# ishine/pix2pixHDAudioSR

Hardware: AMD Instinct MI355X
Metric: MDCT spectrogram frames/sec (G+D fwd+bwd) at 512x256 (higher is better)
Workload: dtype bf16; 1 GPU; configs[1]: ngf=48 n_local_enhancers=0 (GlobalGenerator nd4 nb9) + MultiscaleDiscriminator num_D=2, 512x256 MDCT4 (n_fft 1024, hop 512), LSGAN + feature matching, Adam, bf16 MFMA; per_gpu_batch=32, global_batch=32, parallelism=dp1, launch=hip-graph replay

## Files before the change

pix2pixhdaudiosr_amd/csrc/convplan.h:

```cpp
#pragma once
#include "common.h"
#include <algorithm>

namespace p2phd {

struct GDesc {
  int N, Hin, Win, Cp_in;
  int Hg, Wg;
  int sh, sw, pad_mode;
  int rx_base;
  int Hout, Wout, Cp_out;
  int oh_mul, oh_off, ow_mul, ow_off;
  int Kout, KK, act;
  int nth, ntw, dh0, dh_step, dw0, dw_step;
  int wr0, wr_step, ws0, ws_step;
  int flat_m;
  int cw_inject;
  int cls_cp;
  int n_extent;
  int cls_skip;
  unsigned in_bytes, w_bytes;
  int stats_slots;
  const float* out_scale;
  const void* bs_y;
  const float* bs_stats;
  float* bs_out;
  float bs_inv_hw, bs_eps, bs_slope;
  const void* as_x;
  int grid_m, sk_first, sk_tail, sk_parts, sk_steps;
  float* sk_part;
  unsigned* sk_ticket;
};

struct WMap {
  int rows, inner;
  long s_row, s_inner;
  int row_mod; long s_rowq;
  int c_mod; long s_innerq;
  int S;
  long s_tap;
};
inline WMap plain_map(int rows, int inner, long s_row, long s_inner, int S, long s_tap = 1) {
  return WMap{rows, inner, s_row, s_inner, rows > 0 ? rows : 1, 0, inner > 0 ? inner : 1, 0, S, s_tap};
}

constexpr int P2PHD_FP8_INTERNAL = 2;
int launch_pack_fp8(const GDesc& d, const WMap& m, const float* w, void* wp8, int rows_pad, float* scale2, unsigned* amax_bits,
                    hipStream_t st);

enum LaunchFamily { LC_GCONV = 0, LC_HALO, LC_CLS_SKIP, LC_MARCH, LC_MARCH_W, LC_WGRAD, LC_SPLITK, LC_TILE256, LC_TILE128X192,
                    LC_DFIRST, LC_DLAST, LC_C7, LC_THIN_WGRAD, LC_TIMED_PACK, LC_TIMED_FRAMES, LC_STITCH, LC_PCM, LC_METRICS_ROWS,
                    LC_XOVER, LC_SPECIMG, LC_LOUDNESS, LC_TRUEPEAK, LC_LIMITER, LC_BANDWIDTH, LC_STEREO, LC_RATECONV, LC_FAMILIES };
extern unsigned long long g_launch_count[LC_FAMILIES];

int pcm_check_rows(const char* what, int64_t frames, int channels, int64_t ld, int format, bool encodable);

extern int g_opt_gconv_bm;
extern int g_opt_wgrad_tm;
extern int g_opt_tile128x192;
extern int g_opt_wgrad_xcd;
extern int g_opt_c7_generic;
extern int g_opt_splitk_tail;
extern int g_opt_truepeak_grid;
extern int g_opt_limiter_grid;
extern int g_opt_cus;
int device_cus();
extern int g_opt_reflect_generic;
extern int g_opt_c7_abl;

struct BSum { const void* y; const float* stats; float* out; float inv_hw, eps, slope; };
bool c7_in_shape_ok(const p2phd_conv_desc* c);
size_t c7_in_packed_elems(const p2phd_conv_desc* c);
int c7_in_pack(const p2phd_conv_desc* c, const float* w, void* wf, hipStream_t st);
int c7_in_slots(const p2phd_conv_desc* c);
int c7_in_fwd(const p2phd_conv_desc* c, const void* x, const void* wf, const float* bias, void* y, float* table, hipStream_t st);
bool c7_out_shape_ok(const p2phd_conv_desc* c);
size_t c7_out_packed_elems(const p2phd_conv_desc* c);
int c7_out_pack(const p2phd_conv_desc* c, const float* w, void* wf, hipStream_t st);
int c7_out_fwd(const p2phd_conv_desc* c, const void* x, const void* wf, const float* bias, int act, void* y, hipStream_t st);
bool c7_dgrad_shape_ok(const p2phd_conv_desc* c);
size_t c7_out_dgrad_packed_elems(const p2phd_conv_desc* c);
int c7_out_dgrad_pack(const p2phd_conv_desc* c, const float* w, void* wf, hipStream_t st);
int c7_out_dgrad(const p2phd_conv_desc* c, const void* dy, const void* wf, const float* w_master, void* dx, hipStream_t st);
extern int g_opt_dfirst;
bool dfirst_shape_ok(const p2phd_conv_desc* c);
size_t dfirst_packed_elems(const p2phd_conv_desc* c);
int dfirst_pack(const p2phd_conv_desc* c, const float* w, void* wf, hipStream_t st);
int dfirst_fwd(const p2phd_conv_desc* c, const void* x, const void* wf, const float* bias, int act, void* y, hipStream_t st);
extern int g_opt_dlast;
bool dlast_shape_ok(const p2phd_conv_desc* c);
size_t dlast_packed_elems(const p2phd_conv_desc* c, int which);
int dlast_pack(const p2phd_conv_desc* c, int which, const float* w, void* wfrag, hipStream_t st);
size_t dlast_fwd_workspace_floats(const p2phd_conv_desc* c);
int dlast_fwd(const p2phd_conv_desc* c, const void* x, const void* wf, const float* bias, void* y, float* part, hipStream_t st);
void dlast_dgrad_plan(const p2phd_conv_desc* c, int* bpw, int* slots);
size_t dlast_bsum_table_floats(const p2phd_conv_desc* c);
int dlast_dgrad(const p2phd_conv_desc* c, const void* dy, const void* wg, const void* addend, void* dx, const BSum* bs, hipStream_t st);
extern int g_opt_march; extern int g_opt_cls_skip; extern int g_opt_gconv_halo; extern int g_opt_cw_inject;
int march_shape_kind(const p2phd_conv_desc* c, int which);
size_t march_packed_elems(const p2phd_conv_desc* c, int which);
int march_pack(const p2phd_conv_desc* c, int which, const float* w, void* wf, hipStream_t st);
void march_plan(const p2phd_conv_desc* c, int which, int* slots, int* ncls, int* slot_rows, long* npix_cls, int* bs_tiles);
int march_run(const p2phd_conv_desc* c, int which, const void* in, const void* wf, const float* bias, void* out, float* table,
              const BSum* bs, hipStream_t st, const float* in_stats = nullptr, float in_slope = 1.f, float in_eps = 0.f);
size_t march_w_workspace_floats(const p2phd_conv_desc* c);
int march_w_run(const p2phd_conv_desc* c, const void* x, const void* dy, float* dw, int accumulate, const float* x_stats, float x_slope,
                float x_eps, float* slabs, hipStream_t st);
int thin_wgrad_shape_kind(const p2phd_conv_desc* c);
size_t thin_wgrad_workspace_floats(const p2phd_conv_desc* c);
int thin_wgrad(const p2phd_conv_desc* c, const void* x, const void* dy, float* dw, int accumulate, float* slabs, hipStream_t st);

inline int cpitch(int c) { return (c + 7) & ~7; }
inline int round_up(int v, int m) { return (v + m - 1) / m * m; }

int launch_gconv(const GDesc& d, int dtype, const void* in, const void* wp, const float* bias, const void* addend,
                 void* out, float* stats, hipStream_t st, int* slot_rows = nullptr);
struct GconvTile { int bm, bn, mr, nr, nstage, halo, flat_m; };
GconvTile gconv_choose_tile(const GDesc& d, int dtype, bool stats_wanted);
constexpr int kGconvRows256 = 256, kGconvCols192 = 192;
long gconv_mtiles256(const GDesc& d, bool flat_m);
bool gconv_256x192_fills_chip(const GDesc& d, bool flat_m);
inline int gconv_slot_rows(int bm, int mr, bool fused_sums) { return fused_sums ? bm : mr * 32; }
inline size_t stat_table_floats(const GDesc& d) {
  return (size_t)d.N * ((d.Hg * d.Wg + 31) / 32) * (d.cls_cp > 0 ? 4 : 1) * d.Cp_out * 2;
}
inline size_t bsum_table_floats(const GDesc& d) {
  const size_t tiles = ((size_t)d.Hg * d.Wg + 127) / 128;
  return (size_t)d.N * tiles * (size_t)(d.n_extent ? d.n_extent : d.Cp_out) * 2;
}
int launch_bsum_merge(const float* table, float* bstats, int N, long npix, int tile_rows, int n_extent, int cls_cp, int Cp, int C,
                      hipStream_t st);
int launch_stats_merge(const float* table, float* stats, int N, int slots, int ncls, int Cp, int C, long npix, int slot_rows,
                       hipStream_t st);
size_t wgrad_workspace_floats(const GDesc& d, int dtype, int M_rows, int M_rows_pad);
int launch_wgrad(const GDesc& d, const WMap& m, int dtype, const void* rows, int Cp_r, int M_rows, int M_rows_pad,
                 const void* gat, float* dwp, float* dw, int accumulate, hipStream_t st);
void launch_unpack_grad(const GDesc& d, const WMap& m, const float* dwp, float* dw, int splits, long slab_elems, int accumulate,
                        hipStream_t st);
int launch_pack_merged(const GDesc& d, int dtype, const float* w, void* wp, int rows_pad, int K, int C, int R, int S, int pad,
                       long s_k, long s_c, hipStream_t st);
int launch_pack(const GDesc& d, const WMap& m, int dtype, const float* w, void* wp, int rows_pad, hipStream_t st);
int launch_reflect_expand(int dtype, const void* dy, void* e_out, int N, int H, int W, int Cp, hipStream_t st);
// ... 14 lines not shown
```

pix2pixhdaudiosr_amd/csrc/core.hip:

```cpp
#include "common.h"
#include "convplan.h"
#include <cstring>

namespace p2phd {
static thread_local char g_err[512] = "";
void set_error(const char* fmt, ...) {
  va_list ap;
  va_start(ap, fmt);
  vsnprintf(g_err, sizeof(g_err), fmt, ap);
  va_end(ap);
}
}

namespace p2phd { int g_opt_gconv_bm = 0; int g_opt_wgrad_tm = 0; int g_opt_wgrad_xcd = 1; int g_opt_march = 1; int g_opt_cls_skip = 1; int g_opt_gconv_halo = 1; int g_opt_cw_inject = 0; int g_opt_tile128x192 = 1; int g_opt_mdct_generic = 0; int g_opt_mdct_iters = 0; int g_opt_c7_generic = 0; int g_opt_dfirst = 1; int g_opt_dlast = 1; int g_opt_c7_abl = 0; int g_opt_reflect_generic = 0; int g_opt_splitk_tail = 1; int g_opt_truepeak_grid = 0; int g_opt_limiter_grid = 0; int g_opt_cus = 0;
unsigned long long g_launch_count[LC_FAMILIES] = {};
int device_cus() {
  static int cached[64] = {};
  int dev = 0;
  if (hipGetDevice(&dev) != hipSuccess || dev < 0 || dev >= 64) return 256;
  if (cached[dev] == 0) {
    hipDeviceProp_t prop;
    cached[dev] = hipGetDeviceProperties(&prop, dev) == hipSuccess ? prop.multiProcessorCount : 256;
  }
  return cached[dev];
}
}

namespace {
constexpr int kFoldRegions = 9;
constexpr size_t kFoldFloats[kFoldRegions] = {size_t(4) << 20, size_t(1) << 20, size_t(1) << 20, 4096, size_t(16) << 20, size_t(5) << 16, size_t(1) << 16, size_t(1) << 16, 0};
constexpr int kFoldTickets[kFoldRegions] = {2048, 1024, 8, 8, 256, 8, 8, 8, 1024};
constexpr int kFoldTicketsAll = 2048 + 1024 + 16 + 256 + 8 + 8 + 8 + 1024;
__device__ float g_fold_part[(size_t(22) << 20) + 4096 + (size_t(7) << 16)];
__device__ unsigned g_fold_ticket[kFoldTicketsAll];
}
namespace p2phd {
namespace {
struct FoldDev { float* part = nullptr; unsigned* ticket = nullptr; hipStream_t last[kFoldRegions] = {}; bool used[kFoldRegions] = {}; hipEvent_t ev[kFoldRegions] = {}; bool ev_set[kFoldRegions] = {}; };
FoldDev g_fold_dev[64];
thread_local hipStream_t g_fold_pending_stream = nullptr;
FoldDev* fold_dev() {
  int dev = 0;
  if (hipGetDevice(&dev) != hipSuccess || dev < 0 || dev >= 64) return nullptr;
  FoldDev& f = g_fold_dev[dev];
  if (f.part == nullptr) {
    void* p = nullptr; void* t = nullptr;
    if (hipGetSymbolAddress(&p, HIP_SYMBOL(g_fold_part)) != hipSuccess || hipGetSymbolAddress(&t, HIP_SYMBOL(g_fold_ticket)) != hipSuccess)
      return nullptr;
    f.part = static_cast<float*>(p); f.ticket = static_cast<unsigned*>(t);
  }
  return &f;
}
bool capturing(hipStream_t s) {
  hipStreamCaptureStatus cs = hipStreamCaptureStatusNone;
  return hipStreamIsCapturing(s, &cs) == hipSuccess && cs == hipStreamCaptureStatusActive;
}
}

thread_local int g_fold_pending = -1;

FoldScratch fold_capacity(int region) {
  if (region < 0 || region >= kFoldRegions) return FoldScratch{nullptr, nullptr, 0, 0};
  return FoldScratch{nullptr, nullptr, kFoldFloats[region], kFoldTickets[region]};
}

FoldScratch fold_scratch(int region, hipStream_t stream) {
  FoldDev* f = fold_dev();
  if (f == nullptr || region < 0 || region >= kFoldRegions) { set_error("reduction scratch unavailable"); return FoldScratch{nullptr, nullptr, 0, 0}; }
  const bool cap = capturing(stream);
  if (f->used[region] && f->last[region] != stream && f->ev_set[region] && !cap) {
    if (hipStreamWaitEvent(stream, f->ev[region], 0) != hipSuccess) {
      (void)hipGetLastError();
      set_error("reduction-scratch region %d: cannot order this stream behind the region's previous launch "
                "(include/p2phd.h, \"Streams\")", region);
      return FoldScratch{nullptr, nullptr, 0, 0};
    }
  }
  f->used[region] = true;
  f->last[region] = stream;
  g_fold_pending = cap ? -1 : region;
  g_fold_pending_stream = stream;
  size_t fo = 0; int to = 0;
  for (int r = 0; r < region; ++r) { fo += kFoldFloats[r]; to += kFoldTickets[r]; }
  const FoldScratch cap_of = fold_capacity(region);
  return FoldScratch{f->part + fo, f->ticket + to, cap_of.floats, cap_of.tickets};
}

void fold_launched() {
  const int region = g_fold_pending;
  g_fold_pending = -1;
  FoldDev* f = fold_dev();
  if (f == nullptr || region < 0 || region >= kFoldRegions) return;
  if (f->ev[region] == nullptr && hipEventCreateWithFlags(&f->ev[region], hipEventDisableTiming) != hipSuccess) { (void)hipGetLastError(); f->ev[region] = nullptr; return; }
  if (hipEventRecord(f->ev[region], g_fold_pending_stream) == hipSuccess) f->ev_set[region] = true;
  else (void)hipGetLastError();
}
}

extern "C" int p2phd_reduction_reset(void* stream) {
  void* t = nullptr;
  if (hipGetSymbolAddress(&t, HIP_SYMBOL(g_fold_ticket)) != hipSuccess) { p2phd::set_error("reduction_reset: no device symbol"); return P2PHD_ELAUNCH; }
  if (hipMemsetAsync(t, 0, sizeof(unsigned) * kFoldTicketsAll, (hipStream_t)stream) != hipSuccess) {
    p2phd::set_error("reduction_reset: memset failed");
    return P2PHD_ELAUNCH;
  }
  return P2PHD_OK;
}

extern "C" int p2phd_set_option(const char* name, int value) {
  if (name && !strcmp(name, "gconv_bm") && (value == 0 || value == 128 || value == 192 || value == 256 || value == 258 || value == 512)) { p2phd::g_opt_gconv_bm = value; return P2PHD_OK; }
  if (name && !strcmp(name, "wgrad_tm") && (value == 0 || value == 128)) { p2phd::g_opt_wgrad_tm = value; return P2PHD_OK; }
  if (name && !strcmp(name, "march") && (value == 0 || value == 1)) { p2phd::g_opt_march = value; return P2PHD_OK; }
  if (name && !strcmp(name, "cls_skip") && (value == 0 || value == 1)) { p2phd::g_opt_cls_skip = value; return P2PHD_OK; }
  if (name && !strcmp(name, "gconv_halo") && (value == 0 || value == 1)) { p2phd::g_opt_gconv_halo = value; return P2PHD_OK; }
  if (name && !strcmp(name, "tile128x192") && (value == 0 || value == 1)) { p2phd::g_opt_tile128x192 = value; return P2PHD_OK; }
  if (name && !strcmp(name, "dlast") && (value == 0 || value == 1)) { p2phd::g_opt_dlast = value; return P2PHD_OK; }
  if (name && !strcmp(name, "dfirst") && (value == 0 || value == 1)) { p2phd::g_opt_dfirst = value; return P2PHD_OK; }
#ifdef P2PHD_CHECK_WAITS
  if (name && !strcmp(name, "cw_inject") && (value == 0 || value == 1)) { p2phd::g_opt_cw_inject = value; return P2PHD_OK; }
#endif
  if (name && !strcmp(name, "wgrad_xcd") && (value == 0 || value == 1)) { p2phd::g_opt_wgrad_xcd = value; return P2PHD_OK; }
  if (name && !strcmp(name, "reflect_generic") && (value == 0 || value == 1)) { p2phd::g_opt_reflect_generic = value; return P2PHD_OK; }
  if (name && !strcmp(name, "mdct_iters") && value >= 0 && value <= 8) { p2phd::g_opt_mdct_iters = value; return P2PHD_OK; }
  if (name && !strcmp(name, "splitk_tail") && value >= 0 && value <= 2) { p2phd::g_opt_splitk_tail = value; return P2PHD_OK; }
  if (name && !strcmp(name, "cus") && value >= 0 && value <= 4096) { p2phd::g_opt_cus = value; return P2PHD_OK; }
  if (name && !strcmp(name, "truepeak_grid") && value >= 0 && value <= 65536) { p2phd::g_opt_truepeak_grid = value; return P2PHD_OK; }
  if (name && !strcmp(name, "limiter_grid") && value >= 0 && value <= 16384) { p2phd::g_opt_limiter_grid = value; return P2PHD_OK; }
  if (name && !strcmp(name, "c7_abl")) { p2phd::g_opt_c7_abl = value; return P2PHD_OK; }
  if (name && !strcmp(name, "c7_generic") && (value == 0 || value == 1)) { p2phd::g_opt_c7_generic = value; return P2PHD_OK; }
  if (name && !strcmp(name, "mdct_generic") && (value == 0 || value == 1)) { p2phd::g_opt_mdct_generic = value; return P2PHD_OK; }
  p2phd::set_error("set_option: unknown option or value (%s = %d)", name ? name : "(null)", value);
  return P2PHD_EINVAL;
}

extern "C" int64_t p2phd_launch_count(const char* family, int reset) {
  static const char* names[p2phd::LC_FAMILIES] = {"gconv", "halo", "cls_skip", "march", "march_w", "wgrad", "splitk", "tile256", "tile128x192",
                                                       "dfirst", "dlast", "c7", "thin_wgrad", "timed_pack", "timed_frames", "stitch", "pcm",
                                                       "metrics_rows", "xover", "specimg", "loudness", "truepeak", "limiter", "bandwidth", "stereo", "rateconv"};
  if (family == nullptr) {
    if (reset) for (auto& c : p2phd::g_launch_count) c = 0;
    return 0;
  }
  for (int i = 0; i < p2phd::LC_FAMILIES; ++i)
    if (!strcmp(family, names[i])) {
      const int64_t v = (int64_t)p2phd::g_launch_count[i];
      if (reset) p2phd::g_launch_count[i] = 0;
      return v;
    }
  p2phd::set_error("launch_count: unknown kernel family %s", family);
  return -1;
}

extern "C" const char* p2phd_last_error(void) { return p2phd::g_err; }
extern "C" int p2phd_abi_version(void) { return 1; }
extern "C" int p2phd_half_type(void) {
#ifdef P2PHD_F16
  return 2;
#else
  return 1;
#endif
}

extern "C" int p2phd_device_info(char* name, int cap) {
  int dev = 0;
  if (hipGetDevice(&dev) != hipSuccess) {
    p2phd::set_error("no HIP device");
    return P2PHD_ELAUNCH;
  }
  hipDeviceProp_t prop;
  if (hipGetDeviceProperties(&prop, dev) != hipSuccess) {
    p2phd::set_error("hipGetDeviceProperties failed");
    return P2PHD_ELAUNCH;
  }
  if (name && cap > 0) {
    strncpy(name, prop.gcnArchName, cap - 1);
    name[cap - 1] = 0;
  }
  return prop.multiProcessorCount;
}
```

pix2pixhdaudiosr_amd/csrc/gconv.hip:

```cpp
#include "common.h"
#include "convplan.h"
#include "convdev.h"
#include "waitcheck.h"
#include <cmath>
#include <utility>
#include <vector>
#include <type_traits>

namespace {

using p2phd::GDesc;
using p2phd::GconvTile;

struct fp8_t { unsigned char v; };
template <> struct Elem<fp8_t> { static constexpr int EPP = 16; };
template <typename T> struct OutOf { typedef T type; };
template <> struct OutOf<fp8_t> { typedef bf16_t type; };

#ifdef P2PHD_PROBE
constexpr int kProbeSlots = 65536;
__device__ unsigned long long g_probe[kProbeSlots * 8];
#endif

template <typename T, int BM, int BN, int MR, int NR, int NSTAGE, int HALO = 0>
__global__ __launch_bounds__((BM / (MR * 32)) * (BN / (NR * 32)) * 64) void gconv_kernel(const GDesc d, const T* __restrict__ in, const T* __restrict__ wp,
                                                    const float* __restrict__ bias,
                                                    const typename OutOf<T>::type* __restrict__ addend,
                                                    typename OutOf<T>::type* __restrict__ out, float* __restrict__ stats) {
  typedef typename OutOf<T>::type TO;
  constexpr int EPPO = Elem<TO>::EPP;
  constexpr int EPP = Elem<T>::EPP;
  constexpr int BK = 8 * EPP;
  constexpr int WGM = BM / (MR * 32), WGN = BN / (NR * 32);
  constexpr int NT = WGM * WGN * 64;
  static_assert(NT == BM * 2 || NT == BM, "tile config");
  constexpr int STAGE = (BM + BN) * kRowBytes;
  constexpr int RS = NT / 8;
  constexpr int NB = BN * 8 / NT;
  constexpr int NA = BM * 8 / NT;
  static_assert(NB >= 1 && (NA == 4 || NA == 8), "piece distribution");
  constexpr int NLOADS = NA + NB;

  const int Cp = d.Cp_in, KK = d.KK, Wg = d.Wg, T_taps = d.nth * d.ntw, npix = d.Hg * d.Wg;
  const int Cp_out = d.Cp_out, Kout = d.Kout, act = d.act, cls_cp = d.cls_cp, n_extent = d.n_extent, stats_slots = d.stats_slots;

  extern __shared__ float4 smem_raw[];
  char* smem = reinterpret_cast<char*>(smem_raw);
  int* tab = reinterpret_cast<int*>(smem);
  int2* rinfo = reinterpret_cast<int2*>(smem + (HALO ? 0 : ((T_taps * BM * 4 + 15) & ~15)));
  char* stages = reinterpret_cast<char*>(rinfo + BM);
#ifdef P2PHD_PROBE
  const unsigned long long pr_t0 = __builtin_readcyclecounter();
#endif

  const int tid = threadIdx.x, lane = tid & 63;
  const int wave = __builtin_amdgcn_readfirstlane(tid >> 6);
  const int wm = wave / WGN, wn = wave % WGN;
  const bool flat = d.flat_m != 0;
  const int mtiles = (npix + BM - 1) / BM;
  int tile_id = (int)blockIdx.x, sk_part = -1, sk_tile = 0;
  if (tile_id >= d.sk_first) {
    const int r = tile_id - d.sk_first;
    sk_part = r / d.sk_tail;
    sk_tile = r - sk_part * d.sk_tail;
    tile_id = d.sk_first + sk_tile;
  }
  const int bx = tile_id % d.grid_m;
  int by = tile_id / d.grid_m;
  if (d.cls_skip != 0) by = (d.n_extent + BN - 1) / BN - 1 - by;
  const int n = flat ? 0 : bx / mtiles;
  const int p_base = flat ? bx * BM : (bx - n * mtiles) * BM;
  const int p_end = flat ? d.N * npix : npix;
  const int n0 = by * BN;

  f32x16 acc[MR][NR];
#pragma unroll
  for (int i = 0; i < MR; ++i)
#pragma unroll
    for (int j = 0; j < NR; ++j)
#pragma unroll
      for (int e = 0; e < 16; ++e) acc[i][j][e] = 0.f;
  const int lr = lane & 31, lh = lane >> 5;
#ifdef P2PHD_PROBE
  unsigned long long pr_t1_ = 0, pr_wait_ = 0, pr_bar_ = 0, pr_comp_ = 0;
  int nsteps_ = 0;
#ifdef P2PHD_PROBE_FINE
  unsigned long long pf_a = 0, pf_b = 0;
#endif
#endif
  if constexpr (HALO != 0) {
#include "gconv_halo.inc"
  } else {
  {
    const int Hin = d.Hin, Win = d.Win, sh = d.sh, sw = d.sw, ntw = d.ntw, pad_mode = d.pad_mode;
    const int dh0 = d.dh0, dhs = d.dh_step, dw0 = d.dw0, dws = d.dw_step;
    const int r = tid % BM;
    int p = p_base + r, nn = -1, ho = 0, wo = 0;
    if (p < p_end) {
      nn = n;
      if (flat) { nn = p / npix; p -= nn * npix; }
      ho = p / Wg; wo = p - ho * Wg;
    }
    if (tid < BM) rinfo[r] = make_int2(nn, (ho << 16) | wo);
    constexpr int TPR = NT / BM;
    int ta = 0, tb = tid / BM;
    while (tb >= ntw) { tb -= ntw; ++ta; }
    const bool swap_taps = d.cls_skip != 0 && ((n0 / cls_cp) >> 1) == 1;
    for (int t = tid / BM; t < T_taps; t += TPR) {
      if (swap_taps) { ta = t & 1; tb = t >> 1; }
      int off = -1;
      if (nn >= 0) {
        int hi = ho * sh + dh0 + ta * dhs;
        int wi = wo * sw + dw0 + tb * dws;
        if (pad_mode == 1) { hi = reflect_idx(hi, Hin); wi = reflect_idx(wi, Win); }
        if (pad_mode == 2) {
          const int Hr = Hin - 2, Wr = Win - 2;
          if (ho == 1 && hi == 2) hi = Hr; else if (ho == Hr - 2 && hi == Hr - 3) hi = Hr + 1; else if (hi >= Hr) hi = -1;
          if (wo == 1 && wi == 2) wi = Wr; else if (wo == Wr - 2 && wi == Wr - 3) wi = Wr + 1; else if (wi >= Wr) wi = -1;
        }
        if (pad_mode == 3) {
          const int Hr = Hin, Wr = Win;
          if (ho == 1 && hi == 2) hi = Hr; else if (ho == Hr - 2 && hi == Hr - 3) hi = Hr + 1; else if (hi >= Hr) hi = -1;
          if (wo == 1 && wi == 2) wi = Wr; else if (wo == Wr - 2 && wi == Wr - 3) wi = Wr + 1; else if (wi >= Wr) wi = -1;
          if (hi >= 0 && wi >= 0) {
            if (hi < Hr && wi < Wr) off = (nn * Hr + hi) * Wr + wi;
            else off = d.rx_base + nn * (2 * (Wr + 2) + 2 * Hr) + (hi >= Hr ? (hi - Hr) * (Wr + 2) + wi : 2 * (Wr + 2) + (wi - Wr) * Hr + hi);
          }
        } else if (hi >= 0 && hi < Hin && wi >= 0 && wi < Win) off = (nn * Hin + hi) * Win + wi;
      }
      tab[t * BM + r] = off;
      tb += TPR;
      while (tb >= ntw) { tb -= ntw; ++ta; }
    }
  }
  __syncthreads();
#ifdef P2PHD_PROBE_FINE
  pf_a = __builtin_readcyclecounter();
#endif

  constexpr unsigned kOOB = 0xFFFFFFF0u;
  constexpr int SZ = (int)sizeof(T);
  const int rbase = tid >> 3;
  const int kchunk = (tid & 7) ^ ((rbase >> 1) & 7);
  const int CpB = Cp * SZ;
  int nsteps_all = KK / BK;
  if (d.cls_skip != 0) {
    const int cls_hi = min(3, (n0 + BN - 1) / cls_cp);
    const int ktaps = ((cls_hi >> 1) + 1) * ((cls_hi & 1) + 1);
    nsteps_all = min(nsteps_all, (ktaps * Cp + BK - 1) / BK);
  }
  const int s_begin = sk_part < 0 ? 0 : sk_part * d.sk_steps;
  const int nsteps = sk_part < 0 ? nsteps_all : min(d.sk_steps, nsteps_all - s_begin);
  int a_t, a_cB;
  {
    const long kb = (long)kchunk * EPP * SZ + (long)s_begin * kRowBytes;
    a_t = (int)(kb / CpB);
    a_cB = (int)(kb - (long)a_t * CpB);
  }
  int cur_t = -1;
  unsigned aoffb[NA], va[NA];
#pragma unroll
  for (int i = 0; i < NA; ++i) aoffb[i] = kOOB;
  unsigned boffb[NB];
#pragma unroll
  for (int i = 0; i < NB; ++i) boffb[i] = (unsigned)(((size_t)(n0 + rbase + RS * i) * KK + kchunk * EPP) * SZ);
  const unsigned tab_base = (unsigned)(uintptr_t)(__attribute__((address_space(3))) int*)tab;
  typedef __attribute__((address_space(3))) void* lds_ptr;
  const auto rsA = __builtin_amdgcn_make_buffer_rsrc((void*)in, 0, (int)d.in_bytes, 0x00020000);
  const auto rsB = __builtin_amdgcn_make_buffer_rsrc((void*)wp, 0, (int)d.w_bytes, 0x00020000);

  auto prepare = [&]() {
    if (a_t != cur_t) {
      cur_t = a_t;
      if (a_t < T_taps) {
        int ro[NA];
        const unsigned ta = tab_base + (unsigned)(a_t * BM + rbase) * 4u;
#pragma unroll
        for (int i = 0; i < NA; ++i) asm volatile("ds_read_b32 %0, %1" : "=v"(ro[i]) : "v"(ta + (unsigned)(RS * i * 4)));
        asm volatile("s_waitcnt lgkmcnt(0)" ::: "memory");
        __builtin_amdgcn_sched_barrier(0);
#pragma unroll
        for (int i = 0; i < NA; ++i) aoffb[i] = ro[i] >= 0 ? (unsigned)ro[i] * (unsigned)CpB : kOOB;
      } else {
#pragma unroll
        for (int i = 0; i < NA; ++i) aoffb[i] = kOOB;
      }
    }
#pragma unroll
    for (int i = 0; i < NA; ++i) va[i] = aoffb[i] == kOOB ? kOOB : aoffb[i] + (unsigned)a_cB;
    a_cB += kRowBytes;
    while (a_cB >= CpB) { a_cB -= CpB; ++a_t; }
  };
  P2PHD_CW_DECL;
  auto issue_piece = [&](int slot, int tile, int j) {
    char* A = stages + slot * STAGE + (8 * wave) * kRowBytes;
    P2PHD_CW_ISSUE(slot);
    if (j < NA) {
      __builtin_amdgcn_raw_ptr_buffer_load_lds(rsA, (lds_ptr)(A + RS * j * kRowBytes), 16, (int)va[j], 0, 0, 0);
    } else {
      char* B = A + BM * kRowBytes;
      __builtin_amdgcn_raw_ptr_buffer_load_lds(rsB, (lds_ptr)(B + RS * (j - NA) * kRowBytes), 16, (int)boffb[j - NA],
                                               tile * kRowBytes, 0, 0);
    }
  };

  unsigned fa[MR], fb[NR];
  {
#pragma unroll
    for (int i = 0; i < MR; ++i) {
      const int row = wm * (MR * 32) + i * 32 + lr;
      fa[i] = row * kRowBytes + ((lh ^ ((row >> 1) & 7)) << 4);
    }
#pragma unroll
    for (int j = 0; j < NR; ++j) {
      const int row = wn * (NR * 32) + j * 32 + lr;
      fb[j] = BM * kRowBytes + row * kRowBytes + ((lh ^ ((row >> 1) & 7)) << 4);
    }
  }
  const unsigned frag_base = (unsigned)(uintptr_t)(__attribute__((address_space(3))) char*)stages;

  constexpr int NFB = sizeof(T) == 1 ? 4 : 2;
  uint4 af[NFB][MR], bfr[NFB][NR];
  auto read_frags = [&](unsigned so_, int ks, int buf) {
    const unsigned so = so_ + frag_base;
#pragma unroll
    for (int i = 0; i < MR; ++i) asm volatile("ds_read_b128 %0, %1" : "=v"(af[buf][i]) : "v"((fa[i] ^ (unsigned)(ks << 5)) + so));
#pragma unroll
    for (int j = 0; j < NR; ++j) asm volatile("ds_read_b128 %0, %1" : "=v"(bfr[buf][j]) : "v"((fb[j] ^ (unsigned)(ks << 5)) + so));
  };
  auto mfma_one = [&](int buf, int i, int j) {
    if constexpr (sizeof(T) == 1) {
      (void)buf; (void)i; (void)j;
    } else if constexpr (sizeof(T) == 2) {
      acc[i][j] = p2phd_mfma_32x32x16(*reinterpret_cast<bf16x8*>(&af[buf][i]),
                                                          *reinterpret_cast<bf16x8*>(&bfr[buf][j]), acc[i][j]);
    } else {
      const f32x4 a4 = *reinterpret_cast<f32x4*>(&af[buf][i]);
      const f32x4 b4 = *reinterpret_cast<f32x4*>(&bfr[buf][j]);
#pragma unroll
      for (int e = 0; e < 4; ++e) acc[i][j] = __builtin_amdgcn_mfma_f32_32x32x2f32(a4[e], b4[e], acc[i][j], 0, 0, 0);
    }
  };
  constexpr int NT8 = MR * NR, H1 = NT8;
  auto mfma8 = [&](int ks, int p) {
    if constexpr (sizeof(T) == 1) {
      const int idx = (ks & 1) ? p : H1 + p;
      if (p < H1 && idx < NT8) {
        const int lo = (ks & 1) ? ks - 1 : ((ks + 2) & 3), hi = lo + 1;
        const int i = idx / NR, j = idx % NR;
        typedef __attribute__((ext_vector_type(8))) int i32x8;
        const uint4 a0 = af[lo][i], a1 = af[hi][i], b0 = bfr[lo][j], b1 = bfr[hi][j];
        const i32x8 av = {(int)a0.x, (int)a0.y, (int)a0.z, (int)a0.w, (int)a1.x, (int)a1.y, (int)a1.z, (int)a1.w};
        const i32x8 bv = {(int)b0.x, (int)b0.y, (int)b0.z, (int)b0.w, (int)b1.x, (int)b1.y, (int)b1.z, (int)b1.w};
        acc[i][j] = __builtin_amdgcn_mfma_scale_f32_32x32x64_f8f6f4(av, bv, acc[i][j], 0, 0, 0, 0x7F7F7F7F, 0, 0x7F7F7F7F);
      }
    }
  };
  constexpr bool kScaled = sizeof(T) == 1;
  if constexpr (kScaled) {
#pragma unroll
    for (int i = 0; i < MR; ++i) af[2][i] = af[3][i] = make_uint4(0, 0, 0, 0);
#pragma unroll
    for (int j = 0; j < NR; ++j) bfr[2][j] = bfr[3][j] = make_uint4(0, 0, 0, 0);
  }
  auto mfma_rest = [&](int buf, int skip) {
#pragma unroll
    for (int i = 0; i < MR; ++i)
#pragma unroll
      for (int j = 0; j < NR; ++j)
        if (i * NR + j >= skip) mfma_one(buf, i, j);
  };

#pragma unroll
  for (int t = 0; t < NSTAGE; ++t) {
// ... 308 lines not shown
      for (int t = tid; t < 2 * BN; t += NT) {
        const int col = t >> 1, which = t & 1, pc = col / EPPO, e = col - pc * EPPO;
        float sum = 0.f;
        for (int rg = 0; rg < RG; ++rg) sum += red[(rg * CPR + pc) * (2 * EPPO) + which * EPPO + e];
        if (n0 + col < n_extent)
          d.bs_out[(((size_t)n * mtiles + tile_in_sample) * n_extent + n0 + col) * 2 + which] = sum;
      }
      return;
    }
  }
  {
    constexpr int TOTAL = BM * CPR, U = 4;
    for (int q0 = tid; q0 < TOTAL; q0 += NT * U) {
      int2 ri[U];
      int rowu[U], pcu[U];
#pragma unroll
      for (int u = 0; u < U; ++u) {
        const int q = min(q0 + u * NT, TOTAL - 1);
        rowu[u] = q / CPR; pcu[u] = q - rowu[u] * CPR;
        ri[u] = rinfo[rowu[u]];
      }
      uint4 v[U], av[U];
      size_t off[U];
      bool ok[U];
#pragma unroll
      for (int u = 0; u < U; ++u) {
        int k = n0 + pcu[u] * EPPO;
        ok[u] = q0 + u * NT < TOTAL && ri[u].x >= 0 && k < n_extent;
        int ho = ri[u].y >> 16, wo = ri[u].y & 0xFFFF;
        if (cls_cp > 0) {
          const int cls = (k >= cls_cp) + (k >= 2 * cls_cp) + (k >= 3 * cls_cp);
          k -= cls * cls_cp;
          ho = 2 * ho + (cls >> 1); wo = 2 * wo + (cls & 1);
          ok[u] = ok[u] && ho < Hout && wo < Wout;
        }
        off[u] = ok[u] ? (((size_t)ri[u].x * Hout + (ho * ohm + oho)) * Wout + (wo * owm + owo)) * Cp_out + k : 0;
        v[u] = *reinterpret_cast<const uint4*>(ct + rowu[u] * CROW + pcu[u] * 16);
        if (addend != nullptr) av[u] = *reinterpret_cast<const uint4*>(addend + off[u]);
      }
#pragma unroll
      for (int u = 0; u < U; ++u) {
        if (addend != nullptr) {
          TO* vv = reinterpret_cast<TO*>(&v[u]);
          const TO* aa = reinterpret_cast<const TO*>(&av[u]);
#pragma unroll
          for (int e = 0; e < EPPO; ++e) vv[e] = from_f<TO>(to_f(vv[e]) + to_f(aa[e]));
        }
        if (ok[u]) *reinterpret_cast<uint4*>(out + off[u]) = v[u];
      }
    }
  }
#ifdef P2PHD_PROBE
#ifdef P2PHD_PROBE_DRAIN
  asm volatile("s_waitcnt vmcnt(0)" ::: "memory");
#endif
  const unsigned long long pr_t3 = __builtin_readcyclecounter();
  if (tid == 0) {
    const unsigned wg = (unsigned)blockIdx.x % kProbeSlots;
    unsigned long long* r = g_probe + (size_t)wg * 8;
#ifdef P2PHD_PROBE_FINE
    r[0] += pf_a - pr_t0; r[1] += pf_b - pf_a; r[2] += pr_t1_ - pf_b; r[3] += pr_t2 - pr_t1_;
    r[4] += pf_c - pr_t2; r[5] += pf_d - pf_c; r[6] += 1ull; r[7] += pr_t3 - pf_d;
#else
    r[0] += pr_wait_; r[1] += pr_bar_; r[2] += pr_comp_; r[3] += (unsigned long long)nsteps_;
    r[4] += pr_t1_ - pr_t0; r[5] += pr_t3 - pr_t2; r[6] += 1ull; r[7] += pr_t3 - pr_t0;
#endif
  }
#endif
}

struct GconvProbe {
  bool on = false;
  int cp = 0, kk = 0, hg = 0, wg = 0;
  int pad_mode = -1, esize = 0;
  std::vector<std::pair<hipEvent_t, hipEvent_t>> ev;
};
GconvProbe g_probe_cfg;

template <typename T, int BM, int BN, int MR, int NR, int NSTAGE, int HALO = 0>
int launch_gconv_cfg(const GDesc& d_in, const void* in, const void* wp, const float* bias, const void* addend, void* out,
                     float* stats, hipStream_t st, int* slot_rows) {
  GDesc d = d_in;
  d.stats_slots = (d.Hg * d.Wg + MR * 32 - 1) / (MR * 32);
  if (slot_rows) *slot_rows = p2phd::gconv_slot_rows(BM, MR, d.bs_out != nullptr);
  constexpr int STAGE = (BM + BN) * kRowBytes;
  constexpr int CT = BM * (BN * (int)sizeof(typename OutOf<T>::type) + 16);
  const int tab = (HALO ? 0 : ((d.nth * d.ntw * BM * 4 + 15) & ~15)) + BM * 8;
  constexpr int RING = HALO ? 2 * (20 * 20 * kRowBytes) + 2 * BN * kRowBytes : NSTAGE * STAGE;
  const size_t lds = tab + (size_t)(RING > CT ? RING : CT);
  auto kern = gconv_kernel<T, BM, BN, MR, NR, NSTAGE, HALO>;
  if (lds > 64 * 1024)
    (void)hipFuncSetAttribute(reinterpret_cast<const void*>(kern), hipFuncAttributeMaxDynamicSharedMemorySize, (int)lds);
  const int npix = d.Hg * d.Wg;
  const int mtiles = d.flat_m ? (int)(((long)d.N * npix + BM - 1) / BM) : ((npix + BM - 1) / BM) * d.N;
  const int ntiles = (d.n_extent + BN - 1) / BN;
  const int TT = mtiles * ntiles;
  d.grid_m = mtiles;
  d.sk_first = TT; d.sk_tail = 1; d.sk_parts = 1; d.sk_steps = 0; d.sk_part = nullptr; d.sk_ticket = nullptr;
  int wgs = TT;
  const int cus = p2phd::g_opt_cus > 0 ? p2phd::g_opt_cus : p2phd::device_cus();
  if (p2phd::g_opt_splitk_tail != 0 && d.cls_skip == 0 && HALO == 0) {
    const int nsteps = d.KK / (8 * Elem<T>::EPP);
    const int full = TT / cus * cus, tail = TT - full;
    const double area = (double)BM * BN / 65536.0;
    const double t_slab = (double)BM * BN * 128.0 / 6.0e6, c0 = 8.0 + 16.0 * area, c_io = 4.0 * area;
    const double t_tile = c0 + nsteps * t_slab;
    const double now = (double)(full / cus) * t_tile + (tail > 0 ? 0.75 * t_tile : 0.0);
    int bestP = 1;
    double best = now;
    const int pmax = tail > 0 ? std::min(cus / tail, nsteps / 4) : 1;
    for (int P = 2; P <= pmax; ++P) {
      const int steps = (nsteps + P - 1) / P;
      const int Pe = (nsteps + steps - 1) / steps;
      const double t = (double)(full / cus) * t_tile + c0 + steps * t_slab + c_io + Pe * c_io;
      if (t < best) { best = t; bestP = Pe; }
    }
    if (p2phd::g_opt_splitk_tail == 2 && pmax >= 2) {
      const int steps = (nsteps + pmax - 1) / pmax;
      bestP = (nsteps + steps - 1) / steps;
      best = 0.0;
    }
    if (bestP >= 2 && best < 0.95 * now) {
      const p2phd::FoldScratch fs = p2phd::fold_scratch(p2phd::FOLD_GCONV, st);
      const int steps = (nsteps + bestP - 1) / bestP;
      if (fs.part != nullptr && (size_t)tail * bestP * BM * BN <= fs.floats && tail <= fs.tickets) {
        d.sk_first = full; d.sk_tail = tail; d.sk_parts = bestP; d.sk_steps = steps; d.sk_part = fs.part; d.sk_ticket = fs.ticket;
        wgs = full + tail * bestP;
      }
    }
  }
#ifdef P2PHD_CHECK_WAITS
  d.cw_inject = p2phd::g_opt_cw_inject;
#endif
  dim3 grid((unsigned)wgs);
  const bool probe = g_probe_cfg.on && d.Cp_in == g_probe_cfg.cp && d.KK == g_probe_cfg.kk && d.Hg == g_probe_cfg.hg &&
                     d.Wg == g_probe_cfg.wg && (g_probe_cfg.pad_mode < 0 || d.pad_mode == g_probe_cfg.pad_mode) &&
                     (g_probe_cfg.esize == 0 || (int)sizeof(T) == g_probe_cfg.esize) && g_probe_cfg.ev.size() < 4096;
  hipEvent_t e0 = nullptr, e1 = nullptr;
  if (probe) { (void)hipEventCreate(&e0); (void)hipEventCreate(&e1); (void)hipEventRecord(e0, st); }
  typedef typename OutOf<T>::type TO;
  hipLaunchKernelGGL(kern, grid, dim3((BM / (MR * 32)) * (BN / (NR * 32)) * 64), lds, st, d, (const T*)in, (const T*)wp, bias, (const TO*)addend, (TO*)out, stats);
  ++p2phd::g_launch_count[p2phd::LC_GCONV];
  if (HALO != 0) ++p2phd::g_launch_count[p2phd::LC_HALO];
  if (d.cls_skip != 0) ++p2phd::g_launch_count[p2phd::LC_CLS_SKIP];
  if (d.sk_parts > 1) ++p2phd::g_launch_count[p2phd::LC_SPLITK];
  if (BM == 256 && BN == 256) ++p2phd::g_launch_count[p2phd::LC_TILE256];
  if (BM == 128 && BN == 192) ++p2phd::g_launch_count[p2phd::LC_TILE128X192];
  if (probe) { (void)hipEventRecord(e1, st); g_probe_cfg.ev.emplace_back(e0, e1); }
  return p2phd::check_launch("gconv");
}

typedef int (*GconvLaunch)(const GDesc&, const void*, const void*, const float*, const void*, void*, float*, hipStream_t, int*);
struct GconvRow { int bm, bn, mr, nr, nstage, halo; GconvLaunch launch; };
#define GCONV_ROW(T, BM, BN, MR, NR, NS, HALO) {BM, BN, MR, NR, NS, HALO, launch_gconv_cfg<T, BM, BN, MR, NR, NS, HALO>}
#define GCONV_ROWS_EVERY_TYPE(T) \
  GCONV_ROW(T, 128, 128, 2, 2, 2, 0), GCONV_ROW(T, 128, 64, 2, 1, 2, 0), GCONV_ROW(T, 128, 32, 1, 1, 2, 0), \
  GCONV_ROW(T, 256, 128, 2, 2, 3, 0), GCONV_ROW(T, 256, 128, 2, 2, 2, 0), GCONV_ROW(T, 256, 64, 2, 1, 3, 0), GCONV_ROW(T, 256, 64, 2, 1, 2, 0)
const GconvRow kTilesF32[] = {GCONV_ROWS_EVERY_TYPE(float)};
const GconvRow kTilesFp8[] = {GCONV_ROWS_EVERY_TYPE(fp8_t), GCONV_ROW(fp8_t, 256, 192, 2, 3, 2, 0)};
const GconvRow kTiles16[] = {GCONV_ROWS_EVERY_TYPE(bf16_t), GCONV_ROW(bf16_t, 256, 192, 2, 3, 2, 0), GCONV_ROW(bf16_t, 256, 256, 4, 2, 2, 0),
                             GCONV_ROW(bf16_t, 256, 192, 2, 3, 2, 1), GCONV_ROW(bf16_t, 256, 128, 2, 2, 2, 1), GCONV_ROW(bf16_t, 128, 192, 2, 3, 2, 0)};
#undef GCONV_ROWS_EVERY_TYPE
#undef GCONV_ROW

template <size_t ROWS>
int launch_gconv_tile(const GconvRow (&table)[ROWS], int dtype, GDesc d, const void* in, const void* wp, const float* bias, const void* addend,
                      void* out, float* stats, hipStream_t st, int* slot_rows) {
  if (d.n_extent == 0) d.n_extent = d.Cp_out;
  const GconvTile t = p2phd::gconv_choose_tile(d, dtype, stats != nullptr);
  if (t.bm == 0) return P2PHD_EINVAL;
  d.flat_m = t.flat_m;
  for (const GconvRow& r : table)
    if (r.bm == t.bm && r.bn == t.bn && r.mr == t.mr && r.nr == t.nr && r.nstage == t.nstage && r.halo == t.halo)
      return r.launch(d, in, wp, bias, addend, out, stats, st, slot_rows);
  p2phd::set_error("gconv: no %d x %d tile (waves %d x %d, %d ring slots, halo %d) for dtype %d", t.bm, t.bn, t.mr, t.nr, t.nstage, t.halo, dtype);
  return P2PHD_EINVAL;
}

}

namespace p2phd {

namespace {
struct LdsBudget {
  long tables;
  explicit LdsBudget(int taps) : tables((long)taps * 256 * 4 + 16 + 256 * 8) {}
  bool holds(long bytes) const { return bytes + tables <= 160 * 1024; }
  bool ring(int slots, int bn) const { return holds((long)slots * (256 + bn) * kRowBytes); }
  bool c_tile(int bn, int out_bytes) const { return holds(256 * ((long)bn * out_bytes + 16)); }
};

constexpr double kWgsPerRound = 256.0;
double rounds(long wgs, double per_round) { return std::ceil(wgs / per_round); }

bool gconv_halo_ok(const GDesc& d, bool flat_m) {
  const bool taps = d.nth == 3 && d.ntw == 3 && d.sh == 1 && d.sw == 1 &&
                    ((d.dh0 == -1 && d.dh_step == 1) || (d.dh0 == 1 && d.dh_step == -1)) &&
                    ((d.dw0 == -1 && d.dw_step == 1) || (d.dw0 == 1 && d.dw_step == -1));
  return g_opt_gconv_halo != 0 && taps && d.cls_cp == 0 && d.Wg == 16 && d.Hg % 16 == 0 && d.Hg >= 16 && d.Hin == d.Hg && d.Win == d.Wg &&
         d.Cp_in % 64 == 0 && d.KK == 9 * d.Cp_in && (d.pad_mode == 0 || d.pad_mode == 1 || d.pad_mode == 3) && !flat_m &&
         d.oh_mul == 1 && d.ow_mul == 1 && d.oh_off == 0 && d.ow_off == 0;
}
}

long gconv_mtiles256(const GDesc& d, bool flat_m) {
  const int npix = d.Hg * d.Wg;
  return flat_m ? ((long)d.N * npix + 255) / 256 : (long)((npix + 255) / 256) * d.N;
}

bool gconv_256x192_fills_chip(const GDesc& d, bool flat_m) {
  return gconv_mtiles256(d, flat_m) * ((d.n_extent ? d.n_extent : d.Cp_out) / kGconvCols192) >= 192;
}

GconvTile gconv_choose_tile(const GDesc& d, int dtype, bool stats_wanted) {
  const bool h16 = dtype == P2PHD_BF16, fp8 = dtype == P2PHD_FP8_INTERNAL, f32 = !h16 && !fp8;
  const int epp = fp8 ? 16 : (h16 ? 8 : 4), out_bytes = f32 ? 4 : 2;
  const int k = d.n_extent ? d.n_extent : d.Cp_out;
  if (d.cls_skip != 0) {
    if (h16) return GconvTile{256, 192, 2, 3, 2, 0, 0};
    set_error("gconv: a tap-skipping merged plan reached a non-16-bit launch");
    return GconvTile{};
  }
  const int force = g_opt_gconv_bm;
  const bool fused = d.bs_out != nullptr || d.as_x != nullptr;
  const int npix = d.Hg * d.Wg;
  const bool flat_m = !stats_wanted && d.bs_out == nullptr && npix % 256 != 0;
  const long mt256 = gconv_mtiles256(d, flat_m);
  const LdsBudget lds(d.nth * d.ntw);
  const int bn = k > 64 ? 128 : (k > 32 ? 64 : 32);

// ... 132 lines not shown
```

Baseline: 345,100 frames/s.

## Compute gconv A-operand tap offsets arithmetically instead of via LDS table

For non-halo, zero-padded gconv launches with at most 4x4 taps, the kernel skips building the per-tap LDS offset table. Each row instead keeps a base byte offset and a packed bitmask of valid h/w tap positions, and the tap offset advances incrementally as the K loop walks taps. This removes the table-fill prologue and the LDS reads in the prepare step, at the cost of extra registers per A row. It is enabled by default, with an option to fall back to the table path, and it is counted in a new launch-count family.

```diff
diff --git a/pix2pixhdaudiosr_amd/csrc/convplan.h b/pix2pixhdaudiosr_amd/csrc/convplan.h
--- a/pix2pixhdaudiosr_amd/csrc/convplan.h
+++ b/pix2pixhdaudiosr_amd/csrc/convplan.h
@@ -15,6 +15,7 @@
   int nth, ntw, dh0, dh_step, dw0, dw_step;
   int wr0, wr_step, ws0, ws_step;
   int flat_m;
+  int tab_free;
   int cw_inject;
   int cls_cp;
   int n_extent;
@@ -48,7 +49,7 @@
 int launch_pack_fp8(const GDesc& d, const WMap& m, const float* w, void* wp8, int rows_pad, float* scale2, unsigned* amax_bits,
                     hipStream_t st);
 
-enum LaunchFamily { LC_GCONV = 0, LC_HALO, LC_CLS_SKIP, LC_MARCH, LC_MARCH_W, LC_WGRAD, LC_SPLITK, LC_TILE256, LC_TILE128X192,
+enum LaunchFamily { LC_GCONV = 0, LC_HALO, LC_CLS_SKIP, LC_MARCH, LC_MARCH_W, LC_WGRAD, LC_SPLITK, LC_TILE256, LC_TILE128X192, LC_TABLEFREE,
                     LC_DFIRST, LC_DLAST, LC_C7, LC_THIN_WGRAD, LC_TIMED_PACK, LC_TIMED_FRAMES, LC_STITCH, LC_PCM, LC_METRICS_ROWS,
                     LC_XOVER, LC_SPECIMG, LC_LOUDNESS, LC_TRUEPEAK, LC_LIMITER, LC_BANDWIDTH, LC_STEREO, LC_RATECONV, LC_FAMILIES };
 extern unsigned long long g_launch_count[LC_FAMILIES];
@@ -58,6 +59,7 @@
 extern int g_opt_gconv_bm;
 extern int g_opt_wgrad_tm;
 extern int g_opt_tile128x192;
+extern int g_opt_gconv_table;
 extern int g_opt_wgrad_xcd;
 extern int g_opt_c7_generic;
 extern int g_opt_splitk_tail;
diff --git a/pix2pixhdaudiosr_amd/csrc/core.hip b/pix2pixhdaudiosr_amd/csrc/core.hip
--- a/pix2pixhdaudiosr_amd/csrc/core.hip
+++ b/pix2pixhdaudiosr_amd/csrc/core.hip
@@ -12,7 +12,7 @@
 }
 }
 
-namespace p2phd { int g_opt_gconv_bm = 0; int g_opt_wgrad_tm = 0; int g_opt_wgrad_xcd = 1; int g_opt_march = 1; int g_opt_cls_skip = 1; int g_opt_gconv_halo = 1; int g_opt_cw_inject = 0; int g_opt_tile128x192 = 1; int g_opt_mdct_generic = 0; int g_opt_mdct_iters = 0; int g_opt_c7_generic = 0; int g_opt_dfirst = 1; int g_opt_dlast = 1; int g_opt_c7_abl = 0; int g_opt_reflect_generic = 0; int g_opt_splitk_tail = 1; int g_opt_truepeak_grid = 0; int g_opt_limiter_grid = 0; int g_opt_cus = 0;
+namespace p2phd { int g_opt_gconv_bm = 0; int g_opt_wgrad_tm = 0; int g_opt_wgrad_xcd = 1; int g_opt_march = 1; int g_opt_cls_skip = 1; int g_opt_gconv_halo = 1; int g_opt_cw_inject = 0; int g_opt_tile128x192 = 1; int g_opt_gconv_table = 0; int g_opt_mdct_generic = 0; int g_opt_mdct_iters = 0; int g_opt_c7_generic = 0; int g_opt_dfirst = 1; int g_opt_dlast = 1; int g_opt_c7_abl = 0; int g_opt_reflect_generic = 0; int g_opt_splitk_tail = 1; int g_opt_truepeak_grid = 0; int g_opt_limiter_grid = 0; int g_opt_cus = 0;
 unsigned long long g_launch_count[LC_FAMILIES] = {};
 int device_cus() {
   static int cached[64] = {};
@@ -114,6 +114,7 @@
   if (name && !strcmp(name, "cls_skip") && (value == 0 || value == 1)) { p2phd::g_opt_cls_skip = value; return P2PHD_OK; }
   if (name && !strcmp(name, "gconv_halo") && (value == 0 || value == 1)) { p2phd::g_opt_gconv_halo = value; return P2PHD_OK; }
   if (name && !strcmp(name, "tile128x192") && (value == 0 || value == 1)) { p2phd::g_opt_tile128x192 = value; return P2PHD_OK; }
+  if (name && !strcmp(name, "gconv_table") && (value == 0 || value == 1)) { p2phd::g_opt_gconv_table = value; return P2PHD_OK; }
   if (name && !strcmp(name, "dlast") && (value == 0 || value == 1)) { p2phd::g_opt_dlast = value; return P2PHD_OK; }
   if (name && !strcmp(name, "dfirst") && (value == 0 || value == 1)) { p2phd::g_opt_dfirst = value; return P2PHD_OK; }
 #ifdef P2PHD_CHECK_WAITS
@@ -134,7 +135,7 @@
 }
 
 extern "C" int64_t p2phd_launch_count(const char* family, int reset) {
-  static const char* names[p2phd::LC_FAMILIES] = {"gconv", "halo", "cls_skip", "march", "march_w", "wgrad", "splitk", "tile256", "tile128x192",
+  static const char* names[p2phd::LC_FAMILIES] = {"gconv", "halo", "cls_skip", "march", "march_w", "wgrad", "splitk", "tile256", "tile128x192", "tablefree",
                                                        "dfirst", "dlast", "c7", "thin_wgrad", "timed_pack", "timed_frames", "stitch", "pcm",
                                                        "metrics_rows", "xover", "specimg", "loudness", "truepeak", "limiter", "bandwidth", "stereo", "rateconv"};
   if (family == nullptr) {
diff --git a/pix2pixhdaudiosr_amd/csrc/gconv.hip b/pix2pixhdaudiosr_amd/csrc/gconv.hip
--- a/pix2pixhdaudiosr_amd/csrc/gconv.hip
+++ b/pix2pixhdaudiosr_amd/csrc/gconv.hip
@@ -91,6 +91,7 @@
   if constexpr (HALO != 0) {
 #include "gconv_halo.inc"
   } else {
+  const bool tfree = d.tab_free != 0;
   {
     const int Hin = d.Hin, Win = d.Win, sh = d.sh, sw = d.sw, ntw = d.ntw, pad_mode = d.pad_mode;
     const int dh0 = d.dh0, dhs = d.dh_step, dw0 = d.dw0, dws = d.dw_step;
@@ -106,7 +107,7 @@
     int ta = 0, tb = tid / BM;
     while (tb >= ntw) { tb -= ntw; ++ta; }
     const bool swap_taps = d.cls_skip != 0 && ((n0 / cls_cp) >> 1) == 1;
-    for (int t = tid / BM; t < T_taps; t += TPR) {
+    if (!tfree) for (int t = tid / BM; t < T_taps; t += TPR) {
       if (swap_taps) { ta = t & 1; tb = t >> 1; }
       int off = -1;
       if (nn >= 0) {
@@ -153,14 +154,50 @@
   const int nsteps = sk_part < 0 ? nsteps_all : min(d.sk_steps, nsteps_all - s_begin);
   int a_t, a_cB;
   {
-    const long kb = (long)kchunk * EPP * SZ + (long)s_begin * kRowBytes;
-    a_t = (int)(kb / CpB);
-    a_cB = (int)(kb - (long)a_t * CpB);
+    const unsigned kb = (unsigned)(kchunk * EPP * SZ) + (unsigned)s_begin * (unsigned)kRowBytes;
+    a_t = (int)(kb / (unsigned)CpB);
+    a_cB = (int)(kb - (unsigned)a_t * (unsigned)CpB);
   }
   int cur_t = -1;
   unsigned aoffb[NA], va[NA];
 #pragma unroll
   for (int i = 0; i < NA; ++i) aoffb[i] = kOOB;
+  unsigned baseB[NA], vmask[(NA + 3) / 4], tapB = 0;
+  int t_i = 0, t_o = 0, nI = 1;
+  unsigned stepI = 0, wrapB = 0;
+  if (tfree) {
+    const int Hin = d.Hin, Win = d.Win, sh = d.sh, sw = d.sw, dh0 = d.dh0, dhs = d.dh_step, dw0 = d.dw0, dws = d.dw_step;
+    const bool swap_taps = d.cls_skip != 0 && ((n0 / cls_cp) >> 1) == 1;
+    const unsigned dhB = (unsigned)(dhs * Win) * (unsigned)CpB, dwB = (unsigned)dws * (unsigned)CpB;
+    const unsigned stepO = swap_taps ? dwB : dhB;
+    stepI = swap_taps ? dhB : dwB;
+    nI = swap_taps ? d.nth : d.ntw;
+    wrapB = stepO - (unsigned)nI * stepI;
+#pragma unroll
+    for (int q = 0; q < (NA + 3) / 4; ++q) vmask[q] = 0u;
+#pragma unroll
+    for (int i = 0; i < NA; ++i) {
+      const int2 ri = rinfo[rbase + RS * i];
+      const int h0 = (ri.y >> 16) * sh + dh0, w0 = (ri.y & 0xFFFF) * sw + dw0;
+      baseB[i] = (unsigned)((ri.x * Hin + h0) * Win + w0) * (unsigned)CpB;
+      unsigned mh = 0u, mw = 0u;
+#pragma unroll
+      for (int a = 0; a < 4; ++a) {
+        mh |= ((unsigned)(h0 + a * dhs) < (unsigned)Hin ? 1u : 0u) << a;
+        mw |= ((unsigned)(w0 + a * dws) < (unsigned)Win ? 1u : 0u) << a;
+      }
+      const unsigned mb = ri.x < 0 ? 0u : (swap_taps ? (mh | (mw << 4)) : (mw | (mh << 4)));
+      vmask[i >> 2] |= mb << (8 * (i & 3));
+    }
+    t_i = a_t;
+    while (t_i >= nI) { t_i -= nI; ++t_o; }
+    tapB = (unsigned)t_o * stepO + (unsigned)t_i * stepI;
+  } else {
+#pragma unroll
+    for (int i = 0; i < NA; ++i) baseB[i] = 0u;
+#pragma unroll
+    for (int q = 0; q < (NA + 3) / 4; ++q) vmask[q] = 0u;
+  }
   unsigned boffb[NB];
 #pragma unroll
   for (int i = 0; i < NB; ++i) boffb[i] = (unsigned)(((size_t)(n0 + rbase + RS * i) * KK + kchunk * EPP) * SZ);
@@ -172,7 +209,14 @@
   auto prepare = [&]() {
     if (a_t != cur_t) {
       cur_t = a_t;
-      if (a_t < T_taps) {
+      if (a_t >= T_taps) {
+#pragma unroll
+        for (int i = 0; i < NA; ++i) aoffb[i] = kOOB;
+      } else if (tfree) {
+        const unsigned sel = (1u << t_i) | (16u << t_o);
+#pragma unroll
+        for (int i = 0; i < NA; ++i) aoffb[i] = ((vmask[i >> 2] >> (8 * (i & 3))) & sel) == sel ? baseB[i] + tapB : kOOB;
+      } else {
         int ro[NA];
         const unsigned ta = tab_base + (unsigned)(a_t * BM + rbase) * 4u;
 #pragma unroll
@@ -181,15 +225,16 @@
         __builtin_amdgcn_sched_barrier(0);
 #pragma unroll
         for (int i = 0; i < NA; ++i) aoffb[i] = ro[i] >= 0 ? (unsigned)ro[i] * (unsigned)CpB : kOOB;
-      } else {
-#pragma unroll
-        for (int i = 0; i < NA; ++i) aoffb[i] = kOOB;
       }
     }
 #pragma unroll
     for (int i = 0; i < NA; ++i) va[i] = aoffb[i] == kOOB ? kOOB : aoffb[i] + (unsigned)a_cB;
     a_cB += kRowBytes;
-    while (a_cB >= CpB) { a_cB -= CpB; ++a_t; }
+    while (a_cB >= CpB) {
+      a_cB -= CpB; ++a_t;
+      ++t_i; tapB += stepI;
+      if (t_i == nI) { t_i = 0; ++t_o; tapB += wrapB; }
+    }
   };
   P2PHD_CW_DECL;
   auto issue_piece = [&](int slot, int tile, int j) {
@@ -664,6 +709,7 @@
                      float* stats, hipStream_t st, int* slot_rows) {
   GDesc d = d_in;
   d.stats_slots = (d.Hg * d.Wg + MR * 32 - 1) / (MR * 32);
+  d.tab_free = HALO == 0 && d.pad_mode == 0 && d.nth <= 4 && d.ntw <= 4 && p2phd::g_opt_gconv_table == 0;
   if (slot_rows) *slot_rows = p2phd::gconv_slot_rows(BM, MR, d.bs_out != nullptr);
   constexpr int STAGE = (BM + BN) * kRowBytes;
   constexpr int CT = BM * (BN * (int)sizeof(typename OutOf<T>::type) + 16);
@@ -728,6 +774,7 @@
   if (d.sk_parts > 1) ++p2phd::g_launch_count[p2phd::LC_SPLITK];
   if (BM == 256 && BN == 256) ++p2phd::g_launch_count[p2phd::LC_TILE256];
   if (BM == 128 && BN == 192) ++p2phd::g_launch_count[p2phd::LC_TILE128X192];
+  if (d.tab_free != 0) ++p2phd::g_launch_count[p2phd::LC_TABLEFREE];
   if (probe) { (void)hipEventRecord(e1, st); g_probe_cfg.ev.emplace_back(e0, e1); }
   return p2phd::check_launch("gconv");
 }
```

New measurement: 345,400 frames/s, median of 6. No clear change (+0.1%).
